# bacon205/Multimodal_eeg_fmri

Hardware: AMD Instinct MI355X
Metric: pairs_per_sec_per_node (higher is better)
Workload: dtype bf16

## Files before the change

include/mmeeg_hip.h:

```cpp
#ifndef MMEEG_HIP_H
#define MMEEG_HIP_H

#include <stdint.h>

#ifdef __cplusplus
extern "C" {
#endif

typedef struct ihipStream_t* hipStream_t;

#define MM_ABI_VERSION 5

const char* mm_last_error(void);
int mm_abi_version(void);

int mm_pack_nct_bf16(const float* x, void* y, int B, int C, int T, int Cp, hipStream_t stream);
int mm_unpack_ntc_f32(const void* g, float* dx, int B, int C, int T, int Cp, hipStream_t stream);
int mm_prep_conv_weight(const float* w, void* w_fwd, void* w_dgrad, int Cout, int Cin, int k,
                        int Cinp, int Coutp, hipStream_t stream);

int mm_conv1d_fwd(const void* x, const void* w, int B, int T, int Cin, int Cout, int taps, int pad,
                  const float* scale, const float* shift, int act, const float* residual,
                  const float* pe, int pool, float* stats, float* out_f32, void* out_bf16,
                  void* out_pre, float drop_p, uint32_t drop_seed, const uint32_t* seed_epoch,
// ... 52 lines not shown
                         int B, int D, int H, int W, float drop_p, uint32_t seed, const uint32_t* seed_epoch,
                         hipStream_t stream);
int mm_bn_act_fwd(const float* y, const float* scale, const float* shift, const float* pe,
                  void* out_bf16, float* out_f32, int R, int S, int N, int act, int pool,
                  int drop_first, float drop_p, uint32_t seed, float drop2_p, uint32_t seed2,
                  const uint32_t* seed_epoch, hipStream_t stream);
int mm_bn_act_fwd_ln(const float* y, const float* scale, const float* shift, const float* pe, float* out_f32,
                     int R, int S, int act, float drop_p, uint32_t seed, float drop2_p, uint32_t seed2,
                     const uint32_t* seed_epoch, const float* ln_gamma, const float* ln_beta, float ln_eps,
                     void* ln_out_bf16, float* ln_stat, hipStream_t stream);
int mm_bn_act_bwd_reduce(const float* y, const float* out4, const void* dout_bf16,
                         const float* dout_f32, float* sums_out, int R, int S, int N, int act,
                         int pool, int drop_first, float drop_p, uint32_t seed, float drop2_p,
                         uint32_t seed2, const uint32_t* seed_epoch, hipStream_t stream);
int mm_bn_act_bwd_apply(const float* y, const float* out4, const void* dout_bf16,
                        const float* dout_f32, const float* sums, void* dy, float* dy_f32, int R,
                        int S, int N, int act, int pool, int drop_first, float drop_p, uint32_t seed,
                        float drop2_p, uint32_t seed2, const uint32_t* seed_epoch, int train, int sums_nrep, hipStream_t stream);

int mm_layernorm_fwd(const float* x, const float* gamma, const float* beta, void* out_bf16,
                     float* out_f32, float* stat, int M, int D, float eps, hipStream_t stream);
int mm_layernorm_bwd(const void* dy_bf16, const float* dy_f32, const float* x, const float* stat,
                     const float* gamma, const float* dres, float* dx, void* dx_bf16, float* dgb_repl,
                     int M, int D, float drop_p, uint32_t seed, const uint32_t* seed_epoch,
                     hipStream_t stream);
int mm_linear_dgrad_ln_bwd(const void* dy, const void* w, int M, int K, const float* x, const float* stat,
                           const float* gamma, const float* dres, float* dx, void* dx_bf16, float* dgb_repl,
                           float drop_p, uint32_t seed, const uint32_t* seed_epoch, hipStream_t stream);

int mm_conv1d_dgrad_bn_reduce(const void* dy, const void* w_dgrad, int B, int T, int Cin, int Cout, int taps, int pad,
                              void* dx_bf16, const float* y_below, const float* out4_below, float* sums_below, int act,
                              int pool, int drop_first, float drop_p, uint32_t seed, const uint32_t* seed_epoch,
                              hipStream_t stream);

int mm_linear_fwd_ln_gemm2(const void* x, const void* w, int M, int K, const float* bias, const float* residual,
                           float* out_f32, float drop_p, uint32_t seed, const uint32_t* seed_epoch,
                           const float* ln_gamma, const float* ln_beta, float ln_eps, void* ln_out_bf16, float* ln_stat,
                           const void* w2, const float* bias2, int n2, void* out2_bf16, hipStream_t stream);
int mm_linear_fwd_ln_gemm2_act(const void* x, const void* w, int M, int K, const float* bias, const float* residual,
                               float* out_f32, float drop_p, uint32_t seed, const uint32_t* seed_epoch,
                               const float* ln_gamma, const float* ln_beta, float ln_eps, void* ln_out_bf16,
                               float* ln_stat, const void* w2, const float* bias2, int n2, void* out2_bf16,
                               void* pre2_bf16, int act2, float drop2_p, uint32_t seed2, hipStream_t stream);
int mm_linear_dgrad_ln_bwd_gemm2(const void* dy, const void* w, int M, int K, const float* x, const float* stat,
                                 const float* gamma, const float* dres, float* dx, void* dx_bf16, float* dgb_repl,
                                 float drop_p, uint32_t seed, const uint32_t* seed_epoch, const void* w2, void* do_bf16,
                                 int dres_rows_per_sample, hipStream_t stream);
int mm_linear_dgrad_ln_bwd_bn_reduce(const void* dy, const void* w, int M, int K, const float* x, const float* stat,
                                     const float* gamma, const float* dres, float* dx, float* dgb_repl,
                                     const uint32_t* seed_epoch, const float* y_below, const float* out4_below,
                                     float* sums_below, int act, float bn_drop_p, uint32_t bn_seed, float bn_drop2_p,
                                     uint32_t bn_seed2, hipStream_t stream);

int mm_bn_act_bwd_reduce_bcast(const float* y, const float* out4, const float* dout_rows, float scale, float* sums_out,
                               int R, int S, int N, int act, float drop_p, uint32_t seed, const uint32_t* seed_epoch,
                               hipStream_t stream);
int mm_bn_act_bwd_apply_bcast(const float* y, const float* out4, const float* dout_rows, float scale, const float* sums,
                              void* dy, int R, int S, int N, int act, float drop_p, uint32_t seed,
                              const uint32_t* seed_epoch, int train, int sums_nrep, hipStream_t stream);

int mm_pooled_head_bwd_rows(const float* dout, const void* z_pre_bf16, const float* W, void* dz_bf16, float* rows_out,
                            void* dx_bf16, int B, int L, int D, int N, int act, float drop_p, uint32_t seed,
                            float emit_drop_p, uint32_t emit_seed, const uint32_t* seed_epoch, hipStream_t stream);

int mm_attn_fwd(const void* qkv, void* out, float* lse, int B, int L, int H, int head_dim,
                float scale, float drop_p, uint32_t seed, const uint32_t* seed_epoch,
// ... 160 lines not shown
```

multimodal_eeg_fmri_amd/csrc/common.h:

```cpp
#pragma once
#include <hip/hip_runtime.h>
#include <stdint.h>

typedef __bf16 bf16;
typedef __attribute__((ext_vector_type(8))) __bf16 bf16x8;
typedef __attribute__((ext_vector_type(4))) __bf16 bf16x4;
typedef __attribute__((ext_vector_type(2))) __bf16 bf16x2;
typedef __attribute__((ext_vector_type(16))) float f32x16;
typedef __attribute__((ext_vector_type(4))) float f32x4;
typedef __attribute__((ext_vector_type(4))) short s16x4;

#define MM_OK 0
#define MM_ERR_ARG (-1)
#define MM_ERR_LAUNCH (-2)
#define MM_ERR_UNSUPPORTED (-3)

#define MM_ACT_NONE 0
#define MM_ACT_GELU 1
#define MM_ACT_RELU 2
#define MM_ACT_TANH 3
#define MM_ACT_SIGMOID 4

int mm_fail(int code, const char* fmt, ...);
int mm_check_launch(const char* what);
// ... 94 lines not shown
__device__ __forceinline__ uint32_t mm_eff_seed(uint32_t base, const uint32_t* epoch) {
    return epoch ? base ^ (epoch[0] * 0x85EBCA6Bu + 0xC2B2AE35u) : base;
}

template <int ACT, int POOL, class Args>
__device__ __forceinline__ void bn_dz_pair(const Args& a, float y0, float y1, float sc, float sh, float g,
                                           uint32_t i0, uint32_t i1, uint32_t io, float& dz0, float& dz1) {
    const int act = ACT >= 0 ? ACT : a.act;
    const int pool = POOL > 0 ? POOL : a.pool;
    const float z0 = y0 * sc + sh;
    if (pool == 1) {
        float m = a.thresh ? dropout_scale(a.seed, i0, a.thresh, a.inv_keep) : 1.f;
        dz0 = g * m * act_grad(z0, act);
        dz1 = 0.f;
        return;
    }
    const float z1 = y1 * sc + sh;
    float m0 = 1.f, m1 = 1.f;
    bool first;
    if (a.thresh && a.drop_first) {
        float a0 = apply_act(z0, act), a1 = apply_act(z1, act);
        m0 = dropout_scale(a.seed, i0, a.thresh, a.inv_keep);
        m1 = dropout_scale(a.seed, i1, a.thresh, a.inv_keep);
        a0 *= m0; a1 *= m1;
        first = a0 >= a1;
    } else {
        if (a.thresh) g *= dropout_scale(a.seed, io, a.thresh, a.inv_keep);
        first = z0 >= z1;
        if (act != MM_ACT_GELU || fmaxf(z0, z1) < 0.f) first = apply_act(z0, act) >= apply_act(z1, act);
    }
    const float d = g * (first ? m0 : m1) * act_grad(first ? z0 : z1, act);
    dz0 = first ? d : 0.f;
    dz1 = first ? 0.f : d;
}


#define MM_REPL 32
#define MM_ACC_REPL 16
#define MM_ACC_STAT 28
#define MM_ACC_GRAD 40
typedef long long mm_acc_t;
#define MM_ACC_POISON (1ll << 62)
#define MM_ACC_BAD ((mm_acc_t)0x8000000000000000ull)
#define MM_ACC_MAG_LIMIT ((1u << 25) - 16u)
#ifdef __HIPCC__
template <int K> __device__ __forceinline__ void acc_add(mm_acc_t* p, float v) {
    const float f = v * (float)(1ull << K);
    if (fabsf(f) < 36028797018963968.f)
        atomicAdd(reinterpret_cast<unsigned long long*>(p), (unsigned long long)__float2ll_rn(f));
    else
        atomicExch(reinterpret_cast<unsigned long long*>(p), (unsigned long long)MM_ACC_POISON);
}
template <int K> __device__ __forceinline__ mm_acc_t acc_encode(float v) {
    const float f = v * (float)(1ull << K);
    return fabsf(f) < 2305843009213693952.f ? __float2ll_rn(f) : MM_ACC_POISON;
}
__device__ __forceinline__ unsigned acc_mag(mm_acc_t v) {
    const int hi = (int)(v >> 32);
    return (unsigned)(hi < 0 ? ~hi : hi) >> 4;
}
__device__ __forceinline__ mm_acc_t acc_guard(mm_acc_t s, unsigned mag_sum) { return mag_sum >= MM_ACC_MAG_LIMIT ? MM_ACC_BAD : s; }
template <int K> __device__ __forceinline__ float acc_val(mm_acc_t s) {
    const bool bad = (unsigned long long)(s + (1ll << 61)) >= (1ull << 62);
    return bad ? __builtin_nanf("") : (float)s * (1.0f / (float)(1ull << K));
}
__device__ __forceinline__ mm_acc_t* acc_rep(float* ws, int r, size_t n) { return reinterpret_cast<mm_acc_t*>(ws) + (size_t)r * n; }
// ... 71 lines not shown
```

multimodal_eeg_fmri_amd/csrc/elementwise.hip:

```cpp
#include "common.h"

namespace {

__global__ void bn_finalize_kernel(const float* stats, const float* gamma, const float* beta,
                                   float* run_mean, float* run_var, const float* conv_bias,
                                   float* out , int N,
                                   float count, float momentum, float eps, int mode, long long* tracked) {
    const int n = blockIdx.x * blockDim.x + threadIdx.x;
    if (n >= N) return;
    if (mode == 0) {
        MmBnFin f{stats, gamma, beta, run_mean, run_var, out, tracked, count, momentum, eps, N};
        float sc, sh, mean, rstd;
        bn_fin_channel(f, n, true, sc, sh, mean, rstd);
        return;
    }
    const float mean = run_mean[n], var = run_var[n];
    const float rstd = rsqrtf(var + eps);
    const float sc = gamma[n] * rstd;
    const float cb = (mode == 1 && conv_bias) ? conv_bias[n] : 0.f;
    out[n] = sc;
    out[N + n] = beta[n] + (cb - mean) * sc;
    out[2 * N + n] = mean;
    out[3 * N + n] = rstd;
}

struct BnActArgs {
    const float* y; const float* scale; const float* shift; const float* pe;
    bf16* out_bf16; float* out_f32;
    int R, S, N, act, pool, drop_first;
    uint32_t thresh, seed; float inv_keep;
    uint32_t thresh2, seed2; float inv_keep2;
    const uint32_t* epoch;
    const float* ln_gamma = nullptr; const float* ln_beta = nullptr; float ln_eps = 0.f;
    bf16* ln_out = nullptr; float* ln_stat = nullptr;
    MmBnFin fin = {};
};

template <int ACT>
__device__ __forceinline__ float bnact_one(const BnActArgs& a, float y, float sc, float sh, uint32_t idx, bool drop_here) {
    float v = apply_act(y * sc + sh, ACT >= 0 ? ACT : a.act);
    if (drop_here && a.thresh) v *= dropout_scale(a.seed, idx, a.thresh, a.inv_keep);
    return v;
}

template <int ACT = -1, int POOL = 0, bool FIN = false>
__global__ void bn_act_fwd_kernel(BnActArgs a) {
    a.seed = mm_eff_seed(a.seed, a.epoch);
    a.seed2 = mm_eff_seed(a.seed2, a.epoch);
    if (POOL > 0) a.pool = POOL;
    __shared__ __attribute__((aligned(16))) float s_sc[FIN ? 256 : 4], s_sh[FIN ? 256 : 4];
    if (FIN) {
        for (int n = threadIdx.x; n < a.N; n += blockDim.x) {
            float sc, sh, mean, rstd;
            bn_fin_channel(a.fin, n, blockIdx.x == 0, sc, sh, mean, rstd);
            s_sc[n] = sc; s_sh[n] = sh;
        }
        __syncthreads();
    }
    const int So = a.S / a.pool;
    const unsigned nv = a.N / 4;
    const unsigned total = (unsigned)((size_t)a.R * So * nv);
    for (unsigned i = blockIdx.x * blockDim.x + threadIdx.x; i < total; i += gridDim.x * blockDim.x) {
        const unsigned rs = i / nv;
        const int n4 = (int)(i - rs * nv) * 4;
        const int so = a.pe ? (int)(rs % (unsigned)So) : 0;
        const float4 sc = FIN ? *reinterpret_cast<const float4*>(s_sc + n4) : *reinterpret_cast<const float4*>(a.scale + n4);
        const float4 sh = FIN ? *reinterpret_cast<const float4*>(s_sh + n4) : *reinterpret_cast<const float4*>(a.shift + n4);
        float o[4];
        const size_t in0 = (size_t)rs * a.pool * a.N + n4;
        const float4 y0 = *reinterpret_cast<const float4*>(a.y + in0);
        const float scs[4] = {sc.x, sc.y, sc.z, sc.w}, shs[4] = {sh.x, sh.y, sh.z, sh.w};
        const float y0s[4] = {y0.x, y0.y, y0.z, y0.w};
        const size_t oidx = (size_t)i * 4;
        if (a.pool == 2) {
            const float4 y1 = *reinterpret_cast<const float4*>(a.y + in0 + a.N);
            const float y1s[4] = {y1.x, y1.y, y1.z, y1.w};
#pragma unroll
            for (int q = 0; q < 4; ++q) {
                float m;
                const int act = ACT >= 0 ? ACT : a.act;
                const float z0 = y0s[q] * scs[q] + shs[q], z1 = y1s[q] * scs[q] + shs[q];
                if (act == MM_ACT_GELU && !(a.drop_first && a.thresh) && fmaxf(z0, z1) >= 0.f) {
                    m = gelu_erf(fmaxf(z0, z1));
                } else {
                    const float v0 = bnact_one<ACT>(a, y0s[q], scs[q], shs[q], (uint32_t)(in0 + q), a.drop_first);
                    const float v1 = bnact_one<ACT>(a, y1s[q], scs[q], shs[q], (uint32_t)(in0 + a.N + q), a.drop_first);
                    m = fmaxf(v0, v1);
                }
                if (!a.drop_first && a.thresh) m *= dropout_scale(a.seed, (uint32_t)(oidx + q), a.thresh, a.inv_keep);
                o[q] = m;
            }
        } else {
#pragma unroll
            for (int q = 0; q < 4; ++q) o[q] = bnact_one<ACT>(a, y0s[q], scs[q], shs[q], (uint32_t)(in0 + q), true);
        }
        if (a.pe) {
            const float4 p = *reinterpret_cast<const float4*>(a.pe + (size_t)so * a.N + n4);
            o[0] += p.x; o[1] += p.y; o[2] += p.z; o[3] += p.w;
        }
        if (a.thresh2)
#pragma unroll
            for (int q = 0; q < 4; ++q) o[q] *= dropout_scale(a.seed2, (uint32_t)(oidx + q), a.thresh2, a.inv_keep2);
        if (a.out_f32) *reinterpret_cast<float4*>(a.out_f32 + oidx) = make_float4(o[0], o[1], o[2], o[3]);
        if (a.out_bf16) {
            bf16x4 b = {(bf16)o[0], (bf16)o[1], (bf16)o[2], (bf16)o[3]};
            *reinterpret_cast<bf16x4*>(a.out_bf16 + oidx) = b;
        }
        if (a.ln_out) {
            const float mean = half32_sum((o[0] + o[1]) + (o[2] + o[3])) * (1.f / 128.f);
            const float d0 = o[0] - mean, d1 = o[1] - mean, d2 = o[2] - mean, d3 = o[3] - mean;
            const float rstd = rsqrtf(half32_sum((d0 * d0 + d1 * d1) + (d2 * d2 + d3 * d3)) * (1.f / 128.f) + a.ln_eps);
            const float4 g4 = *reinterpret_cast<const float4*>(a.ln_gamma + n4);
            const float4 b4 = *reinterpret_cast<const float4*>(a.ln_beta + n4);
            bf16x4 hv = {(bf16)(d0 * rstd * g4.x + b4.x), (bf16)(d1 * rstd * g4.y + b4.y),
                         (bf16)(d2 * rstd * g4.z + b4.z), (bf16)(d3 * rstd * g4.w + b4.w)};
            *reinterpret_cast<bf16x4*>(a.ln_out + oidx) = hv;
            if (a.ln_stat && n4 == 0) { a.ln_stat[2 * (size_t)rs] = mean; a.ln_stat[2 * (size_t)rs + 1] = rstd; }
        }
    }
}

struct BnBwdArgs {
    const float* y; const float* scale; const float* shift; const float* mean; const float* rstd;
    const bf16* dout_bf16; const float* dout_f32; const float* sums;
    float* sums_out; bf16* dy; float* dy_f32;
    int R, S, N, act, pool, drop_first, train;
    uint32_t thresh, seed; float inv_keep, inv_count;
// ... 623 lines not shown
```

multimodal_eeg_fmri_amd/csrc/igemm1d.hip:

```cpp
#include "common.h"

#include <cstdio>
#include <cstdlib>

namespace {


constexpr int KPAD = 8;
constexpr int A2S = 128 + KPAD;

struct BnRed {
    const float* y = nullptr;
    const float* out4 = nullptr;
    float* sums = nullptr;
    int act = 0, pool = 1, drop_first = 0;
    uint32_t thresh = 0, seed = 0;
    float inv_keep = 1.f;
    const uint32_t* epoch = nullptr;
    uint32_t thresh2 = 0, seed2 = 0;
    float inv_keep2 = 1.f;
};

struct EpiArgs {
    const float* scale;
    const float* shift;
    const float* residual;
    const float* pe;
    float* stats;
    float* out_f32;
    bf16* out_bf16;
    bf16* out_pre;
    int act;
    int pool;
    uint32_t drop_thresh;
    uint32_t drop_seed;
    float drop_inv_keep;
    const uint32_t* drop_epoch;
    const bf16* gradz;
    int gradz_act;
    const float* ln_x;
    const float* ln_stat;
    const float* ln_gamma;
    float* ln_dgb;
    float* pool_out;
    int pool_rows;
    float pool_scale;
    bf16* lnf_out;
    float* lnf_stat;
    const float* lnf_gamma;
    const float* lnf_beta;
    float lnf_eps;
    BnRed bn;
    const bf16* w2 = nullptr;
    bf16* out2 = nullptr;
    const float* bias2 = nullptr;
    int n2 = 128;
    int act2 = 0;
    uint32_t thresh2 = 0, seed2 = 0; float inv_keep2 = 1.f;
    bf16* pre2 = nullptr;
    int res_rows = 0;
};

struct ConvArgs {
    const bf16* x;
    const bf16* w;
    int B, T, Cin, Cout, taps, pad;
    EpiArgs e;
    float* partial = nullptr;
    int csplit = 0;
};

enum : unsigned { EF_RES = 1, EF_PE = 2, EF_PRE = 4, EF_GRADZ = 8, EF_STATS = 16, EF_POOLOUT = 32, EF_LNF = 64, EF_POOL2 = 128,
                  EF_DROP = 256, EF_SCALE = 512, EF_F32 = 1024, EF_BF16 = 2048, EF_SHIFT = 4096, EF_LNBWD = 8192,
                  EF_BNRED = 16384, EF_BNPOOL2 = 32768 ,
                  EF_GEMM2 = 1u << 28, EF_ANY = 0xFFFFFFFFu };
static unsigned epi_mask(const EpiArgs& e) {
    return (e.residual ? EF_RES : 0) | (e.pe ? EF_PE : 0) | (e.out_pre ? EF_PRE : 0) | (e.gradz ? EF_GRADZ : 0) | (e.stats ? EF_STATS : 0) |
           (e.pool_out ? EF_POOLOUT : 0) | (e.lnf_out ? EF_LNF : 0) | (e.pool == 2 ? EF_POOL2 : 0) | (e.drop_thresh ? EF_DROP : 0) |
           (e.scale ? EF_SCALE : 0) | (e.out_f32 ? EF_F32 : 0) | (e.out_bf16 ? EF_BF16 : 0) | (e.shift ? EF_SHIFT : 0) | (e.ln_x ? EF_LNBWD : 0) |
           ((unsigned)e.act << 16) | ((unsigned)(e.gradz ? e.gradz_act : 0) << 20) |
           (e.bn.y ? (EF_BNRED | (e.bn.pool == 2 ? EF_BNPOOL2 : 0) | ((unsigned)e.bn.act << 24)) : 0) | (e.w2 ? EF_GEMM2 : 0);
}


template <int BM, int BN, unsigned FEAT>
__device__ __forceinline__ void epilogue_rows(const float* Cs, const EpiArgs& e, int tid, int b, int t0, int T,
                                              int n0, int N, float* sstat, bf16* a2 = nullptr) {
#pragma clang fp contract(off)
    constexpr bool ANY = FEAT == EF_ANY;
#define EF_ON(bit, runtime) (ANY ? (bool)(runtime) : ((FEAT & (bit)) != 0))
    const int act = ANY ? e.act : (int)((FEAT >> 16) & 15u);
    const int gradz_act = ANY ? e.gradz_act : (int)((FEAT >> 20) & 15u);
    constexpr int LDC = BN + 4;
    constexpr int CG = BN / 4;
    constexpr int RPP = 256 / CG;
    const int cg = tid % CG, rr = tid / CG;
    const int n = n0 + cg * 4;
    const bool nok = n < N;
    float4 sc = make_float4(1.f, 1.f, 1.f, 1.f), sh = make_float4(0.f, 0.f, 0.f, 0.f);
    if (nok) {
        if (EF_ON(EF_SCALE, e.scale)) sc = *reinterpret_cast<const float4*>(e.scale + n);
        if (EF_ON(EF_SHIFT, e.shift)) sh = *reinterpret_cast<const float4*>(e.shift + n);
    }
    const float scs[4] = {sc.x, sc.y, sc.z, sc.w}, shs[4] = {sh.x, sh.y, sh.z, sh.w};
    float s1[4] = {0, 0, 0, 0}, s2[4] = {0, 0, 0, 0}, pp[4] = {0, 0, 0, 0};
    const bool drop = EF_ON(EF_DROP, e.drop_thresh);
    const uint32_t dseed = drop ? mm_eff_seed(e.drop_seed, e.drop_epoch) : 0u;
    const int step = ANY ? e.pool : ((FEAT & EF_POOL2) ? 2 : 1);
    const int To = T / step;
    for (int r0 = rr * step; r0 < BM; r0 += RPP * step) {
        float o[4] = {-INFINITY, -INFINITY, -INFINITY, -INFINITY};
        bool any = false;
        for (int q = 0; q < step; ++q) {
            const int row = r0 + q, t = t0 + row;
// ... 312 lines not shown
                const size_t idx = (row0 + row) * e.n2 + n;
                const float v = e.bias2 ? c2[r] + bias : c2[r];
                if (e.pre2) e.pre2[idx] = (bf16)v;
                float val = apply_act(v, e.act2);
                if (e.thresh2) val = __builtin_fmaf(val, dropout_scale(dseed, (uint32_t)idx, e.thresh2, e.inv_keep2), 0.f);
                orow[(size_t)row * e.n2] = (bf16)val;
            }
        }
    }
}

template <int BM, int BN, int WM, int WN, int KCT, unsigned FEAT, int TAPS>
__global__ __launch_bounds__(256, 2) void conv1d_fwd_kernel(ConvArgs a) {
    if (TAPS > 0) a.taps = TAPS;
    constexpr int TM = BM / (WM * 32);
    constexpr int TN = BN / (WN * 32);
    static_assert(WM * WN == 4, "4 waves");
    constexpr int AS = KCT + KPAD;
    constexpr int SEGS = KCT / 8;
    extern __shared__ __attribute__((aligned(16))) char smem[];

    const int tid = threadIdx.x;
    const int lane = tid & 63;
    const int wave = tid >> 6;
    const int wm = wave / WN, wn = wave % WN;
    const int tilesT = (a.T + BM - 1) / BM;
    const int b = blockIdx.x / tilesT;
    const int t0 = (blockIdx.x % tilesT) * BM;
    const int n0 = blockIdx.y * BN;
    const int arows = BM + a.taps - 1;
    bf16* As = reinterpret_cast<bf16*>(smem);
    bf16* Ws = As + arows * AS;

    f32x16 acc[TM][TN];
#pragma unroll
    for (int i = 0; i < TM; ++i)
#pragma unroll
        for (int j = 0; j < TN; ++j)
#pragma unroll
            for (int r = 0; r < 16; ++r) acc[i][j][r] = 0.f;

    const bf16* xb = a.x + (size_t)b * a.T * a.Cin;
    const int lr = lane & 31, lh = lane >> 5;
    const int wrows = BN * a.taps;
    const int wvalid = (a.Cout - n0) * a.taps;

    constexpr bool MERGE = BM == 32;
    constexpr int NA = MERGE ? 2 : 4, NB = 8;
    const bf16* wb = a.w + (size_t)n0 * a.taps * a.Cin;
    const int nA = arows * SEGS, nW = wrows * SEGS;
    auto load_a = [&](int s, int c0) {
        const int r = s / SEGS, sg = s % SEGS;
        const int t = t0 - a.pad + r;
        return (s < nA && t >= 0 && t < a.T) ? *reinterpret_cast<const uint4*>(xb + (size_t)t * a.Cin + c0 + sg * 8)
                                             : make_uint4(0, 0, 0, 0);
    };
    auto load_w = [&](int s, int c0) {
        const int r = s / SEGS, sg = s % SEGS;
        return (s < nW && r < wvalid) ? *reinterpret_cast<const uint4*>(wb + (size_t)r * a.Cin + c0 + sg * 8)
                                      : make_uint4(0, 0, 0, 0);
    };
    const int c_lo = a.partial ? (int)blockIdx.z * a.csplit : 0;
    const int c_hi = a.partial ? min(a.Cin, c_lo + a.csplit) : a.Cin;
    for (int c0 = c_lo; c0 < c_hi; c0 += KCT) {
        if (c0 != c_lo) __syncthreads();
        if constexpr (MERGE) {
            uint4 va[NA], vw[NB];
#pragma unroll
            for (int i = 0; i < NA; ++i) va[i] = load_a(i * 256 + tid, c0);
#pragma unroll
            for (int i = 0; i < NB; ++i) vw[i] = load_w(i * 256 + tid, c0);
#pragma unroll
            for (int i = 0; i < NA; ++i) {
                const int s = i * 256 + tid;
                if (s < nA) *reinterpret_cast<uint4*>(As + (s / SEGS) * AS + (s % SEGS) * 8) = va[i];
            }
#pragma unroll
            for (int i = 0; i < NB; ++i) {
                const int s = i * 256 + tid;
                if (s < nW) *reinterpret_cast<uint4*>(Ws + (s / SEGS) * AS + (s % SEGS) * 8) = vw[i];
            }
        }
        for (int base = MERGE ? NA * 256 : 0; base < nA; base += NA * 256) {
            uint4 v[NA];
#pragma unroll
            for (int i = 0; i < NA; ++i) v[i] = load_a(base + i * 256 + tid, c0);
#pragma unroll
            for (int i = 0; i < NA; ++i) {
                const int s = base + i * 256 + tid;
                if (s < nA) *reinterpret_cast<uint4*>(As + (s / SEGS) * AS + (s % SEGS) * 8) = v[i];
            }
        }
        for (int base = MERGE ? NB * 256 : 0; base < nW; base += NB * 256) {
            uint4 v[NB];
#pragma unroll
            for (int i = 0; i < NB; ++i) v[i] = load_w(base + i * 256 + tid, c0);
#pragma unroll
            for (int i = 0; i < NB; ++i) {
                const int s = base + i * 256 + tid;
                if (s < nW) *reinterpret_cast<uint4*>(Ws + (s / SEGS) * AS + (s % SEGS) * 8) = v[i];
            }
        }
        __syncthreads();
        for (int tap = 0; tap < a.taps; ++tap) {
#pragma unroll
            for (int ks = 0; ks < KCT; ks += 16) {
                bf16x8 af[TM], bfr[TN];
#pragma unroll
                for (int i = 0; i < TM; ++i) {
                    const int row = (wm * TM + i) * 32 + lr + tap;
                    af[i] = *reinterpret_cast<const bf16x8*>(As + row * AS + ks + lh * 8);
                }
#pragma unroll
                for (int j = 0; j < TN; ++j) {
                    const int nl = (wn * TN + j) * 32 + lr;
                    bfr[j] = *reinterpret_cast<const bf16x8*>(Ws + (nl * a.taps + tap) * AS + ks + lh * 8);
// ... 774 lines not shown
    a.e.pool_out = nullptr; a.e.pool_rows = 0; a.e.pool_scale = 0.f;
    a.e.lnf_out = nullptr; a.e.lnf_stat = nullptr; a.e.lnf_gamma = nullptr; a.e.lnf_beta = nullptr; a.e.lnf_eps = 0.f;
    return 0;
}

int mm_conv1d_dgrad_bn_reduce(const void* dy, const void* w_dgrad, int B, int T, int Cin, int Cout, int taps, int pad,
                              void* dx_bf16, const float* y_below, const float* out4_below, float* sums_below, int act,
                              int pool, int drop_first, float drop_p, uint32_t seed, const uint32_t* seed_epoch,
                              hipStream_t st) {
    MM_REQUIRE(dy && w_dgrad && dx_bf16 && y_below && out4_below && sums_below, "conv1d_dgrad_bn_reduce: null");
    MM_REQUIRE(B > 0 && T > 0 && Cout > 0 && taps >= 1 && taps <= 9 && pad >= 0 && pad < taps, "conv1d_dgrad_bn_reduce: bad dims");
    MM_REQUIRE(Cin > 0 && Cin % 16 == 0 && Cout % 4 == 0, "conv1d_dgrad_bn_reduce: Cin=%d (x16) Cout=%d (x4)", Cin, Cout);
    MM_REQUIRE(taps > 1 || Cout <= 64, "conv1d_dgrad_bn_reduce: the fused reduce runs on the 64 x 64 tile (taps > 1 or Cout <= 64)");
    MM_REQUIRE(pool == 1 || pool == 2, "conv1d_dgrad_bn_reduce: pool=%d", pool);
    MM_REQUIRE(drop_p >= 0.f && drop_p < 1.f, "conv1d_dgrad_bn_reduce: drop_p");
    MM_REQUIRE((size_t)B * T * pool * Cout < (1ull << 32), "conv1d_dgrad_bn_reduce: 32-bit dropout indices");
    ConvArgs a;
    a.x = (const bf16*)dy; a.w = (const bf16*)w_dgrad;
    a.B = B; a.T = T; a.Cin = Cin; a.Cout = Cout; a.taps = taps; a.pad = pad;
    a.e.scale = nullptr; a.e.shift = nullptr; a.e.residual = nullptr; a.e.pe = nullptr; a.e.stats = nullptr;
    a.e.out_f32 = nullptr; a.e.out_bf16 = (bf16*)dx_bf16; a.e.out_pre = nullptr;
    a.e.act = 0; a.e.pool = 1;
    a.e.drop_thresh = 0u; a.e.drop_seed = 0u; a.e.drop_epoch = nullptr; a.e.drop_inv_keep = 1.f;
    a.e.gradz = nullptr; a.e.gradz_act = 0;
    a.e.ln_x = nullptr; a.e.ln_stat = nullptr; a.e.ln_gamma = nullptr; a.e.ln_dgb = nullptr;
    a.e.pool_out = nullptr; a.e.pool_rows = 0; a.e.pool_scale = 0.f;
    a.e.lnf_out = nullptr; a.e.lnf_stat = nullptr; a.e.lnf_gamma = nullptr; a.e.lnf_beta = nullptr; a.e.lnf_eps = 0.f;
    a.e.bn.y = y_below; a.e.bn.out4 = out4_below; a.e.bn.sums = sums_below;
    a.e.bn.act = act; a.e.bn.pool = pool; a.e.bn.drop_first = drop_first;
    a.e.bn.thresh = drop_p > 0.f ? (uint32_t)((double)drop_p * 4294967296.0) : 0u;
    a.e.bn.seed = seed; a.e.bn.inv_keep = drop_p > 0.f ? 1.f / (1.f - drop_p) : 1.f;
    a.e.bn.epoch = seed_epoch;
    return conv1d_dispatch(a, st);
}

static int linear128_fwd(const void* x, const void* w, int M, int K, const float* bias, const float* residual,
                         float* out_f32, float drop_p, uint32_t seed, const uint32_t* seed_epoch, float* pool_out,
                         int rows_per_group, const float* ln_gamma, const float* ln_beta, float ln_eps, void* ln_out,
                         float* ln_stat, hipStream_t st, const void* w2 = nullptr, const float* bias2 = nullptr, int n2 = 0,
                         void* out2 = nullptr, int act2 = 0, float drop2_p = 0.f, uint32_t seed2 = 0, void* pre2 = nullptr) {
    MM_REQUIRE(x && w && out_f32 && M > 0 && M % 32 == 0 && K > 0 && K % 16 == 0, "linear128_fwd: M=%d (x32) K=%d (x16)", M, K);
    MM_REQUIRE(drop_p >= 0.f && drop_p < 1.f, "linear128_fwd: drop_p");
    MM_REQUIRE(!pool_out || (rows_per_group > 0 && rows_per_group % 32 == 0 && M % rows_per_group == 0),
               "linear128_fwd: rows_per_group=%d must be a multiple of 32 dividing M=%d", rows_per_group, M);
    MM_REQUIRE(!ln_out || (ln_gamma && ln_beta), "linear128_fwd: LayerNorm parameters");
    ConvArgs a;
    a.x = (const bf16*)x; a.w = (const bf16*)w;
    a.B = 1; a.T = M; a.Cin = K; a.Cout = 128; a.taps = 1; a.pad = 0;
    a.e.scale = nullptr; a.e.shift = bias; a.e.residual = residual; a.e.pe = nullptr; a.e.stats = nullptr;
    a.e.out_f32 = out_f32; a.e.out_bf16 = nullptr; a.e.out_pre = nullptr;
    a.e.act = 0; a.e.pool = 1;
    a.e.drop_thresh = drop_p > 0.f ? (uint32_t)((double)drop_p * 4294967296.0) : 0u;
    a.e.drop_seed = seed; a.e.drop_epoch = seed_epoch;
    a.e.drop_inv_keep = drop_p > 0.f ? 1.0f / (1.0f - drop_p) : 1.f;
    a.e.gradz = nullptr; a.e.gradz_act = 0;
    a.e.ln_x = nullptr; a.e.ln_stat = nullptr; a.e.ln_gamma = nullptr; a.e.ln_dgb = nullptr;
    a.e.pool_out = pool_out; a.e.pool_rows = pool_out ? rows_per_group : 0;
    a.e.pool_scale = pool_out ? 1.f / (float)rows_per_group : 0.f;
    a.e.lnf_out = (bf16*)ln_out; a.e.lnf_stat = ln_stat; a.e.lnf_gamma = ln_gamma; a.e.lnf_beta = ln_beta; a.e.lnf_eps = ln_eps;
    if (w2) {
        MM_REQUIRE(ln_out && out2 && n2 > 0 && n2 % 128 == 0, "linear128_fwd: the second GEMM needs the LayerNorm rows, an output and n2 %% 128 == 0 (n2=%d)", n2);
        MM_REQUIRE(drop2_p >= 0.f && drop2_p < 1.f && (size_t)M * n2 < (1ull << 32), "linear128_fwd: second GEMM dropout / 32-bit indices");
        a.e.w2 = (const bf16*)w2; a.e.bias2 = bias2; a.e.n2 = n2; a.e.out2 = (bf16*)out2;
        a.e.act2 = act2; a.e.pre2 = (bf16*)pre2;
        a.e.thresh2 = drop2_p > 0.f ? (uint32_t)((double)drop2_p * 4294967296.0) : 0u;
        a.e.seed2 = seed2; a.e.inv_keep2 = drop2_p > 0.f ? 1.0f / (1.0f - drop2_p) : 1.f;
// ... 338 lines not shown
```

multimodal_eeg_fmri_amd/ops.py:

```python
from __future__ import annotations

import math
import os
import weakref
from typing import Dict, List, Optional, Tuple

import torch

from . import _hip

ACT = {"none": 0, "gelu": 1, "relu": 2, "tanh": 3, "sigmoid": 4}
_BF = torch.bfloat16
_F32 = torch.float32


def _need_gpu(*tensors):
    for t in tensors:
        if t is not None and not t.is_cuda:
            raise _hip.HipLibraryError(
                "multimodal_eeg_fmri_amd runs on the MI355X HIP path only: got a CPU tensor "
                "(no CPU / eager-PyTorch fallback is provided)")
    _hip.load()


# ... 350 lines not shown


ATTN_HEAD_DIMS = tuple(range(16, 65, 8))


def attn_entry(d_model: int, nhead: int, which: str) -> str:
    dh = d_model // nhead if nhead > 0 else 0
    if nhead <= 0 or d_model % nhead or dh not in ATTN_HEAD_DIMS:
        raise ValueError(f"self-attention: (d_model, nhead) = ({d_model}, {nhead}) gives a head dim the kernels do not run; "
                         f"supported head dims: {', '.join(map(str, ATTN_HEAD_DIMS))}")
    return f"mm_attn_{which}" if dh == 32 else f"mm_attn_{which}_hd"


def attn_mask_per_head(mask, B: int, nhead: int, L: int) -> int:
    if mask is None or mask.dim() == 2:
        return 0
    if tuple(mask.shape) != (B * nhead, L, L):
        raise ValueError(f"attn_mask: the 3-D form must be (batch * heads, L, L) = ({B * nhead}, {L}, {L}), got {tuple(mask.shape)}")
    return 1


def additive_attn_mask(mask, L: int, like: torch.Tensor):
    if mask is None:
        return None
    if mask.dim() not in (2, 3) or tuple(mask.shape[-2:]) != (L, L):
        raise ValueError(f"attn_mask: expected (L, L) or (batch * heads, L, L) with L = {L}, got {tuple(mask.shape)}")
    if mask.dtype == torch.bool:
        m = torch.zeros(tuple(mask.shape), dtype=_F32, device=like.device)
        m.masked_fill_(mask.to(like.device), float("-inf"))
        return m
    return mask.to(device=like.device, dtype=_F32).contiguous()


def conv_bn_act(xb: torch.Tensor, conv, bn, *, act="gelu", pool=1, training=False, drop_p=0.0,
                drop_first=True, pe=None, pe_drop_p=0.0, want_f32=False, want_bf16=True, need_dgrad=False,
                save=None, next_norm=None):
    save = training if save is None else save
    k = conv.kernel_size[0]
    pad = conv.padding[0]
    cout = conv.out_channels
    wf, _, cinp, _ = weights.get(conv.weight, need_dgrad)
    assert xb.shape[2] == cinp, (xb.shape, cinp)
    B, T, _ = xb.shape
    if not save:
        out4 = bn_fold_eval(bn, conv.bias)
        r = igemm(xb, wf, k, pad, cout, scale=out4[0], shift=out4[1], act=act, pe=pe, pool=pool,
                  out_f32=want_f32, out_bf16=want_bf16)
        return r, None
    stats = _zeros((REPL, 2, cout), xb) if training else None
    y = igemm(xb, wf, k, pad, cout, shift=conv.bias, stats=stats, out_f32=True, out_bf16=False)["f32"]
    fold = training and act == "gelu" and cout <= 256 and isinstance(bn.running_mean, torch.Tensor)
    fin = None
    if fold:
        fin, out4 = bn_fin_desc(bn, stats, B * T)
    else:
        out4 = bn_finalize_train(bn, stats, B * T) if training else bn_fold_eval(bn, None)
    if not training:
        drop_p = pe_drop_p = 0.0
    seed = _next_seed() if drop_p > 0 else 0
    seed2 = _next_seed() if pe_drop_p > 0 else 0
    of = _empty((B, T // pool, cout), _F32, xb) if want_f32 else None
    ob = _empty((B, T // pool, cout), _BF, xb) if want_bf16 else None
    prenorm = None
    if next_norm is not None and cout == 128 and pool == 1 and want_f32 and not want_bf16 and drop_first \
            and tuple(next_norm.normalized_shape) == (128,):
        hn = _empty((B * T, cout), _BF, xb)
        stn = _empty((B * T, 2), _F32, xb)
        if fold:
            import ctypes
            _hip.call("mm_bn_act_fwd_ln_fin", y, ctypes.addressof(fin), pe, of, B, T, ACT[act], float(drop_p), seed,
                      float(pe_drop_p), seed2, EP(), next_norm.weight, next_norm.bias, float(next_norm.eps), hn, stn)
        else:
            _hip.call("mm_bn_act_fwd_ln", y, out4[0], out4[1], pe, of, B, T, ACT[act], float(drop_p), seed,
                      float(pe_drop_p), seed2, EP(), next_norm.weight, next_norm.bias, float(next_norm.eps), hn, stn)
        prenorm = (hn, stn)
    elif fold:
        import ctypes
        _hip.call("mm_bn_act_fwd_fin", y, ctypes.addressof(fin), pe, ob, of, B, T, cout, ACT[act], pool,
                  1 if drop_first else 0, float(drop_p), seed, float(pe_drop_p), seed2, EP())
    else:
        _hip.call("mm_bn_act_fwd", y, out4[0], out4[1], pe, ob, of, B, T, cout, ACT[act], pool,
                  1 if drop_first else 0, float(drop_p), seed, float(pe_drop_p), seed2, EP())
    saved = dict(xb=xb, y=y, out4=out4, act=act, pool=pool, drop_p=drop_p, seed=seed,
                 drop2=(float(pe_drop_p), seed2), drop_first=drop_first, conv=conv, bn=bn, train=training)
    return {"f32": of, "bf16": ob, "pre": None, "prenorm": prenorm}, saved


def transformer_block_fwd(x: torch.Tensor, blk, training: bool, need_dgrad: bool = False,
                          save: Optional[bool] = None, pool_out: Optional[torch.Tensor] = None,
                          prenorm=None, next_norm=None, mask=None, next_blk=None):
    B, L, D = x.shape
    M = B * L
    save = training if save is None else save
    p = blk.dropout.p if training else 0.0
    x2 = x.view(M, D)
    fuse_ln = D == 128 and M % 32 == 0
    h1, st1 = prenorm[:2] if prenorm is not None else layernorm(x2, blk.norm1, save)
    if prenorm is not None and len(prenorm) > 2:
        qkv = prenorm[2]
    else:
        qkv = linear_rows(h1, blk.self_attn.in_proj_weight, blk.self_attn.in_proj_bias,
                          need_dgrad=need_dgrad)["bf16"]
    pa = float(blk.self_attn.dropout) if training else 0.0
    sa = _next_seed() if pa > 0 else 0
    o, lse = attention(qkv.view(B, L, 3 * D), blk.nhead, save, pa, sa, mask)
    s1 = _next_seed() if p > 0 else 0
    f1 = None
    s2 = None
    if fuse_ln:
        wf, _, cinp, _ = weights.get(blk.self_attn.out_proj.weight, need_dgrad)
        x1 = _empty((M, D), _F32, x)
        h2 = _empty((M, D), _BF, x)
        st2 = _empty((M, 2), _F32, x) if save else None
        w1, _, c1, _ = weights.get(blk.linear1.weight, need_dgrad)
        n1 = blk.linear1.weight.shape[0]
        if c1 == 128 and n1 % 128 == 0 and M * n1 < (1 << 32) and not _NO_FFN1_FUSE:
            s2 = _next_seed() if p > 0 else 0
            g1 = _empty((M, n1), _BF, x)
# ... 88 lines not shown
    if L > pe.shape[0]:
        raise ValueError(f"sequence length {L} exceeds PositionalEncoding max_len {pe.shape[0]}")
    return pe[:L, 0, :].contiguous()


def _encoder_tail_impl(m, h, training: bool, need_dgrad: bool, save: bool, prenorm=None, stages=None):
    blocks = []
    B, L, D = h.shape
    nblk = len(m.transformer_layers)
    pooled = _zeros((B, 2 * D), h) if nblk and L % 32 == 0 and D == 128 else None
    layers = list(m.transformer_layers)
    for i, blk in enumerate(layers):
        if i < nblk - 1:
            h, s, prenorm = transformer_block_fwd(h, blk, training, need_dgrad, save=save, prenorm=prenorm,
                                                  next_norm=layers[i + 1].norm1, next_blk=layers[i + 1])
        else:
            h, s = transformer_block_fwd(h, blk, training, need_dgrad, save=save, pool_out=pooled, prenorm=prenorm)
        blocks.append(s)
        if stages is not None:
            stages[f"block{i}"] = h.clone()
    out, s = pooled_head_fwd(h, m.output_proj[2], training=training, drop_p=m.drop_p, need_dgrad=need_dgrad,
                             save=save, pooled_f32=pooled)
    return out, blocks, s, h


def _erp_forward_impl(m, x: torch.Tensor, training: bool, need_dgrad: bool, save=None, xb=None, stages=None):
    cl = m.conv_layers
    save = training if save is None else save
    p = m.drop_p if training else 0.0
    if xb is None:
        xb = pack_nct(x)
    saved = []
    saved_in = []
    r, s = conv_bn_act(xb, cl[0], cl[1], training=training, drop_p=p, need_dgrad=need_dgrad, save=save)
    saved.append(s)
    saved_in.append(r["bf16"])
    r, s = conv_bn_act(r["bf16"], cl[4], cl[5], pool=2, training=training, drop_p=p,
                       drop_first=False, need_dgrad=need_dgrad, save=save)
    saved.append(s)
    saved_in.append(r["bf16"])
    L = r["bf16"].shape[1]
    r, s = conv_bn_act(r["bf16"], cl[9], cl[10], training=training, drop_p=p,
                       pe=pe_table(m.pos_encoder, L), pe_drop_p=(m.pos_encoder.dropout.p if training else 0.0),
                       want_f32=True, want_bf16=False, need_dgrad=need_dgrad, save=save,
                       next_norm=m.transformer_layers[0].norm1 if len(m.transformer_layers) else None)
    saved.append(s)
    if stages is not None:
        stages["conv1"], stages["conv2"] = saved_in[0].clone(), saved_in[1].clone()
        stages["pos"] = r["f32"].clone()
        if not save:
            wf3 = weights.get(cl[9].weight, need_dgrad)[0]
            o4 = bn_fold_eval(cl[10], cl[9].bias)
            stages["conv3"] = igemm(saved_in[1], wf3, cl[9].kernel_size[0], cl[9].padding[0], cl[9].out_channels,
                                    scale=o4[0], shift=o4[1], act="gelu", out_f32=True, out_bf16=False)["f32"]
    out, blocks, s, h = _encoder_tail_impl(m, r["f32"], training, need_dgrad, save, prenorm=r.get("prenorm"), stages=stages)
    return out, dict(convs=saved, blocks=blocks, head=s, x_shape=tuple(x.shape), tokens=h)


def erp_encoder_forward(m, x: torch.Tensor) -> torch.Tensor:
    _need_gpu(x)
    if m.training or _wants_grad(m, x):
        from .autograd import ErpEncoderFn
        return ErpEncoderFn.run(m, x)
    with torch.no_grad():
        return _erp_forward_impl(m, x.float(), False, False)[0]


def _wants_grad(m, x) -> bool:
    return torch.is_grad_enabled() and (x.requires_grad or any(p.requires_grad for p in m.parameters()))


def add_positional(x, pe, drop_p, training):
    _need_gpu(x)
    if x.dim() != 3:
        raise ValueError("PositionalEncoding: expected a 3-D input (batch, seq, d_model) or (seq, 1, d_model)")
    L = x.size(1) if x.size(1) != 1 else x.size(0)
    if L > pe.shape[0]:
        raise ValueError(f"sequence length {L} exceeds PositionalEncoding max_len {pe.shape[0]}")
    from .autograd import AddPositionalFn
# ... 738 lines not shown
```

Baseline: 41800.

## Fuse BatchNorm apply, GELU, pool and dropout into next conv's input staging

In training, the BN-apply/activation/pool/dropout pass of the first two conv blocks is deferred. The next implicit-GEMM conv then reads the raw fp32 pre-BN output and applies BN finalize, GELU, optional max-pool and dropout while staging its A tile into shared memory. It also writes the bf16 activation once, from blockIdx.y==0 tiles, for the backward pass. This removes a separate elementwise kernel launch and its bf16 round trip per block. In exchange, the conv reads fp32 data (twice as much when pooled) and recomputes the activation for every output-channel tile, and the new path is restricted to 64-row tiles.

```diff
diff --git a/include/mmeeg_hip.h b/include/mmeeg_hip.h
--- a/include/mmeeg_hip.h
+++ b/include/mmeeg_hip.h
@@ -108,6 +108,9 @@
                               void* dx_bf16, const float* y_below, const float* out4_below, float* sums_below, int act,
                               int pool, int drop_first, float drop_p, uint32_t seed, const uint32_t* seed_epoch,
                               hipStream_t stream);
+int mm_conv1d_fwd_bn_in(const float* y_below, const void* bn_fin_host, int pool, int drop_first, float drop_p,
+                        uint32_t seed, void* act_bf16, const void* w, int B, int T, int Cin, int Cout, int taps, int pad,
+                        const float* shift, float* stats, float* out_f32, const uint32_t* seed_epoch, hipStream_t stream);
 
 int mm_linear_fwd_ln_gemm2(const void* x, const void* w, int M, int K, const float* bias, const float* residual,
                            float* out_f32, float drop_p, uint32_t seed, const uint32_t* seed_epoch,
diff --git a/multimodal_eeg_fmri_amd/csrc/common.h b/multimodal_eeg_fmri_amd/csrc/common.h
--- a/multimodal_eeg_fmri_amd/csrc/common.h
+++ b/multimodal_eeg_fmri_amd/csrc/common.h
@@ -150,6 +150,33 @@
     const float d = g * (first ? m0 : m1) * act_grad(first ? z0 : z1, act);
     dz0 = first ? d : 0.f;
     dz1 = first ? 0.f : d;
+}
+
+template <int ACT, int POOL, class Args>
+__device__ __forceinline__ float bn_act_fwd_one(const Args& a, float y0, float y1, float sc, float sh,
+                                                uint32_t i0, uint32_t i1, uint32_t io) {
+    const int act = ACT >= 0 ? ACT : a.act;
+    const int pool = POOL > 0 ? POOL : a.pool;
+    const float z0 = y0 * sc + sh;
+    if (pool == 1) {
+        float v = apply_act(z0, act);
+        if (a.thresh) v *= dropout_scale(a.seed, i0, a.thresh, a.inv_keep);
+        return v;
+    }
+    const float z1 = y1 * sc + sh;
+    float m;
+    if (act == MM_ACT_GELU && !(a.drop_first && a.thresh) && fmaxf(z0, z1) >= 0.f) {
+        m = gelu_erf(fmaxf(z0, z1));
+    } else {
+        float v0 = apply_act(z0, act), v1 = apply_act(z1, act);
+        if (a.drop_first && a.thresh) {
+            v0 *= dropout_scale(a.seed, i0, a.thresh, a.inv_keep);
+            v1 *= dropout_scale(a.seed, i1, a.thresh, a.inv_keep);
+        }
+        m = fmaxf(v0, v1);
+    }
+    if (!a.drop_first && a.thresh) m *= dropout_scale(a.seed, io, a.thresh, a.inv_keep);
+    return m;
 }
 
 
diff --git a/multimodal_eeg_fmri_amd/csrc/elementwise.hip b/multimodal_eeg_fmri_amd/csrc/elementwise.hip
--- a/multimodal_eeg_fmri_amd/csrc/elementwise.hip
+++ b/multimodal_eeg_fmri_amd/csrc/elementwise.hip
@@ -35,13 +35,6 @@
     bf16* ln_out = nullptr; float* ln_stat = nullptr;
     MmBnFin fin = {};
 };
-
-template <int ACT>
-__device__ __forceinline__ float bnact_one(const BnActArgs& a, float y, float sc, float sh, uint32_t idx, bool drop_here) {
-    float v = apply_act(y * sc + sh, ACT >= 0 ? ACT : a.act);
-    if (drop_here && a.thresh) v *= dropout_scale(a.seed, idx, a.thresh, a.inv_keep);
-    return v;
-}
 
 template <int ACT = -1, int POOL = 0, bool FIN = false>
 __global__ void bn_act_fwd_kernel(BnActArgs a) {
@@ -76,23 +69,12 @@
             const float4 y1 = *reinterpret_cast<const float4*>(a.y + in0 + a.N);
             const float y1s[4] = {y1.x, y1.y, y1.z, y1.w};
 #pragma unroll
-            for (int q = 0; q < 4; ++q) {
-                float m;
-                const int act = ACT >= 0 ? ACT : a.act;
-                const float z0 = y0s[q] * scs[q] + shs[q], z1 = y1s[q] * scs[q] + shs[q];
-                if (act == MM_ACT_GELU && !(a.drop_first && a.thresh) && fmaxf(z0, z1) >= 0.f) {
-                    m = gelu_erf(fmaxf(z0, z1));
-                } else {
-                    const float v0 = bnact_one<ACT>(a, y0s[q], scs[q], shs[q], (uint32_t)(in0 + q), a.drop_first);
-                    const float v1 = bnact_one<ACT>(a, y1s[q], scs[q], shs[q], (uint32_t)(in0 + a.N + q), a.drop_first);
-                    m = fmaxf(v0, v1);
-                }
-                if (!a.drop_first && a.thresh) m *= dropout_scale(a.seed, (uint32_t)(oidx + q), a.thresh, a.inv_keep);
-                o[q] = m;
-            }
+            for (int q = 0; q < 4; ++q)
+                o[q] = bn_act_fwd_one<ACT, 2>(a, y0s[q], y1s[q], scs[q], shs[q], (uint32_t)(in0 + q), (uint32_t)(in0 + a.N + q),
+                                              (uint32_t)(oidx + q));
         } else {
 #pragma unroll
-            for (int q = 0; q < 4; ++q) o[q] = bnact_one<ACT>(a, y0s[q], scs[q], shs[q], (uint32_t)(in0 + q), true);
+            for (int q = 0; q < 4; ++q) o[q] = bn_act_fwd_one<ACT, 1>(a, y0s[q], y0s[q], scs[q], shs[q], (uint32_t)(in0 + q), 0u, 0u);
         }
         if (a.pe) {
             const float4 p = *reinterpret_cast<const float4*>(a.pe + (size_t)so * a.N + n4);
diff --git a/multimodal_eeg_fmri_amd/csrc/igemm1d.hip b/multimodal_eeg_fmri_amd/csrc/igemm1d.hip
--- a/multimodal_eeg_fmri_amd/csrc/igemm1d.hip
+++ b/multimodal_eeg_fmri_amd/csrc/igemm1d.hip
@@ -19,6 +19,16 @@
     const uint32_t* epoch = nullptr;
     uint32_t thresh2 = 0, seed2 = 0;
     float inv_keep2 = 1.f;
+};
+
+struct BnIn {
+    const float* y = nullptr;
+    MmBnFin fin = {};
+    bf16* act_out = nullptr;
+    int act = MM_ACT_GELU, pool = 1, drop_first = 1;
+    uint32_t thresh = 0, seed = 0;
+    float inv_keep = 1.f;
+    const uint32_t* epoch = nullptr;
 };
 
 struct EpiArgs {
@@ -59,6 +69,7 @@
     uint32_t thresh2 = 0, seed2 = 0; float inv_keep2 = 1.f;
     bf16* pre2 = nullptr;
     int res_rows = 0;
+    BnIn bnin;
 };
 
 struct ConvArgs {
@@ -73,13 +84,14 @@
 enum : unsigned { EF_RES = 1, EF_PE = 2, EF_PRE = 4, EF_GRADZ = 8, EF_STATS = 16, EF_POOLOUT = 32, EF_LNF = 64, EF_POOL2 = 128,
                   EF_DROP = 256, EF_SCALE = 512, EF_F32 = 1024, EF_BF16 = 2048, EF_SHIFT = 4096, EF_LNBWD = 8192,
                   EF_BNRED = 16384, EF_BNPOOL2 = 32768 ,
-                  EF_GEMM2 = 1u << 28, EF_ANY = 0xFFFFFFFFu };
+                  EF_GEMM2 = 1u << 28, EF_BNIN = 1u << 29, EF_BNIN_POOL2 = 1u << 30, EF_ANY = 0xFFFFFFFFu };
 static unsigned epi_mask(const EpiArgs& e) {
     return (e.residual ? EF_RES : 0) | (e.pe ? EF_PE : 0) | (e.out_pre ? EF_PRE : 0) | (e.gradz ? EF_GRADZ : 0) | (e.stats ? EF_STATS : 0) |
            (e.pool_out ? EF_POOLOUT : 0) | (e.lnf_out ? EF_LNF : 0) | (e.pool == 2 ? EF_POOL2 : 0) | (e.drop_thresh ? EF_DROP : 0) |
            (e.scale ? EF_SCALE : 0) | (e.out_f32 ? EF_F32 : 0) | (e.out_bf16 ? EF_BF16 : 0) | (e.shift ? EF_SHIFT : 0) | (e.ln_x ? EF_LNBWD : 0) |
            ((unsigned)e.act << 16) | ((unsigned)(e.gradz ? e.gradz_act : 0) << 20) |
-           (e.bn.y ? (EF_BNRED | (e.bn.pool == 2 ? EF_BNPOOL2 : 0) | ((unsigned)e.bn.act << 24)) : 0) | (e.w2 ? EF_GEMM2 : 0);
+           (e.bn.y ? (EF_BNRED | (e.bn.pool == 2 ? EF_BNPOOL2 : 0) | ((unsigned)e.bn.act << 24)) : 0) | (e.w2 ? EF_GEMM2 : 0) |
+           (e.bnin.y ? (EF_BNIN | (e.bnin.pool == 2 ? EF_BNIN_POOL2 : 0)) : 0);
 }
 
 
@@ -458,6 +470,19 @@
     bf16* As = reinterpret_cast<bf16*>(smem);
     bf16* Ws = As + arows * AS;
 
+    constexpr bool BNIN = FEAT != EF_ANY && (FEAT & EF_BNIN) != 0;
+    constexpr int BPOOL = (FEAT & EF_BNIN_POOL2) && BNIN ? 2 : 1;
+    __shared__ __attribute__((aligned(16))) float s_bn[BNIN ? 512 : 1];
+    if constexpr (BNIN) {
+        a.e.bnin.seed = mm_eff_seed(a.e.bnin.seed, a.e.bnin.epoch);
+        for (int n = tid; n < a.Cin; n += 256) {
+            float sc, sh, mean, rstd;
+            bn_fin_channel(a.e.bnin.fin, n, blockIdx.x == 0 && blockIdx.y == 0, sc, sh, mean, rstd);
+            s_bn[n] = sc; s_bn[256 + n] = sh;
+        }
+        __syncthreads();
+    }
+
     f32x16 acc[TM][TN];
 #pragma unroll
     for (int i = 0; i < TM; ++i)
@@ -472,6 +497,7 @@
     const int wvalid = (a.Cout - n0) * a.taps;
 
     constexpr bool MERGE = BM == 32;
+    static_assert(!(MERGE && BNIN), "the BatchNorm-applying staging runs on the 64-row tiles");
     constexpr int NA = MERGE ? 2 : 4, NB = 8;
     const bf16* wb = a.w + (size_t)n0 * a.taps * a.Cin;
     const int nA = arows * SEGS, nW = wrows * SEGS;
@@ -486,6 +512,50 @@
         return (s < nW && r < wvalid) ? *reinterpret_cast<const uint4*>(wb + (size_t)r * a.Cin + c0 + sg * 8)
                                       : make_uint4(0, 0, 0, 0);
     };
+    auto stage_bn = [&](int base, int c0) __attribute__((always_inline)) {
+        constexpr int NY = 2 * BPOOL;
+        const int Tin = a.T * BPOOL;
+        const float* yb = a.e.bnin.y + (size_t)b * Tin * a.Cin;
+        float4 v[NA][NY];
+#pragma unroll
+        for (int i = 0; i < NA; ++i) {
+            const int s = base + i * 256 + tid;
+            const int r = s / SEGS, sg = s % SEGS;
+            const int t = t0 - a.pad + r;
+            const bool ok = s < nA && t >= 0 && t < a.T;
+            const float* p = yb + (ok ? (size_t)t * BPOOL * a.Cin + c0 + sg * 8 : 0);
+#pragma unroll
+            for (int j = 0; j < BPOOL; ++j) {
+                v[i][2 * j] = *reinterpret_cast<const float4*>(p + j * a.Cin);
+                v[i][2 * j + 1] = *reinterpret_cast<const float4*>(p + j * a.Cin + 4);
+            }
+        }
+#pragma unroll
+        for (int i = 0; i < NA; ++i) {
+            const int s = base + i * 256 + tid;
+            if (s >= nA) continue;
+            const int r = s / SEGS, sg = s % SEGS;
+            const int t = t0 - a.pad + r;
+            const int c = c0 + sg * 8;
+            bf16x8 h;
+#pragma unroll
+            for (int q = 0; q < 8; ++q) h[q] = (bf16)0.f;
+            if (t >= 0 && t < a.T) {
+                const float y0s[8] = {v[i][0].x, v[i][0].y, v[i][0].z, v[i][0].w, v[i][1].x, v[i][1].y, v[i][1].z, v[i][1].w};
+                const float4 u0 = v[i][NY - 2], u1 = v[i][NY - 1];
+                const float y1s[8] = {u0.x, u0.y, u0.z, u0.w, u1.x, u1.y, u1.z, u1.w};
+                const uint32_t i0 = (uint32_t)(((size_t)b * Tin + (size_t)t * BPOOL) * a.Cin + c);
+                const uint32_t io = (uint32_t)(((size_t)b * a.T + t) * a.Cin + c);
+#pragma unroll
+                for (int q = 0; q < 8; ++q)
+                    h[q] = (bf16)bn_act_fwd_one<MM_ACT_GELU, BPOOL>(a.e.bnin, y0s[q], y1s[q], s_bn[c + q], s_bn[256 + c + q],
+                                                                    i0 + q, i0 + a.Cin + q, io + q);
+                if (blockIdx.y == 0 && r >= a.pad && r < a.pad + BM)
+                    *reinterpret_cast<bf16x8*>(a.e.bnin.act_out + ((size_t)b * a.T + t) * a.Cin + c) = h;
+            }
+            *reinterpret_cast<bf16x8*>(As + r * AS + sg * 8) = h;
+        }
+    };
     const int c_lo = a.partial ? (int)blockIdx.z * a.csplit : 0;
     const int c_hi = a.partial ? min(a.Cin, c_lo + a.csplit) : a.Cin;
     for (int c0 = c_lo; c0 < c_hi; c0 += KCT) {
@@ -508,6 +578,10 @@
             }
         }
         for (int base = MERGE ? NA * 256 : 0; base < nA; base += NA * 256) {
+            if constexpr (BNIN) {
+                stage_bn(base, c0);
+                continue;
+            }
             uint4 v[NA];
 #pragma unroll
             for (int i = 0; i < NA; ++i) v[i] = load_a(base + i * 256 + tid, c0);
@@ -1348,6 +1422,29 @@
     a.e.bn.seed = seed; a.e.bn.inv_keep = drop_p > 0.f ? 1.f / (1.f - drop_p) : 1.f;
     a.e.bn.epoch = seed_epoch;
     return conv1d_dispatch(a, st);
+}
+
+int mm_conv1d_fwd_bn_in(const float* y_below, const void* bn_fin_host, int pool, int drop_first, float drop_p, uint32_t seed,
+                        void* act_bf16, const void* w, int B, int T, int Cin, int Cout, int taps, int pad, const float* shift,
+                        float* stats, float* out_f32, const uint32_t* seed_epoch, hipStream_t st) {
+    MM_REQUIRE(y_below && act_bf16 && shift && stats && out_f32, "conv1d_fwd_bn_in: null");
+    ConvArgs a;
+    int rc = conv1d_fwd_args(a, act_bf16, w, B, T, Cin, Cout, taps, pad, nullptr, shift, 0, nullptr, nullptr, 1, stats, out_f32,
+                             nullptr, nullptr, 0.f, 0u, seed_epoch, nullptr, 0);
+    if (rc) return rc;
+    MM_REQUIRE(bn_fin_from_host(a.e.bnin.fin, bn_fin_host, Cin), "conv1d_fwd_bn_in: incomplete mm_bn_fin_t (null pointer or count < 1)");
+    MM_REQUIRE(taps > 1 && Cin % 64 == 0 && Cin <= 256, "conv1d_fwd_bn_in: taps=%d (> 1), Cin=%d (a multiple of 64, <= 256)", taps, Cin);
+    MM_REQUIRE(conv1d_splitk_slices(B, T, Cin, Cout, taps) == 1, "conv1d_fwd_bn_in: a split-K shape");
+    MM_REQUIRE(pool == 1 || pool == 2, "conv1d_fwd_bn_in: pool=%d", pool);
+    MM_REQUIRE(drop_p >= 0.f && drop_p < 1.f, "conv1d_fwd_bn_in: drop_p");
+    MM_REQUIRE((size_t)B * T * pool * Cin < (1ull << 32), "conv1d_fwd_bn_in: 32-bit dropout indices");
+    a.e.bnin.y = y_below; a.e.bnin.act_out = (bf16*)act_bf16;
+    a.e.bnin.act = MM_ACT_GELU; a.e.bnin.pool = pool; a.e.bnin.drop_first = drop_first ? 1 : 0;
+    a.e.bnin.thresh = drop_p > 0.f ? (uint32_t)((double)drop_p * 4294967296.0) : 0u;
+    a.e.bnin.seed = seed; a.e.bnin.inv_keep = drop_p > 0.f ? 1.f / (1.f - drop_p) : 1.f;
+    a.e.bnin.epoch = seed_epoch;
+    if (pool == 2) return launch_fwd_feat<64, 64, 2, 2, 64, 0x001410u | EF_BNIN | EF_BNIN_POOL2, 0>(a, st);
+    return launch_fwd_feat<64, 64, 2, 2, 64, 0x001410u | EF_BNIN, 0>(a, st);
 }
 
 static int linear128_fwd(const void* x, const void* w, int M, int K, const float* bias, const float* residual,
diff --git a/multimodal_eeg_fmri_amd/ops.py b/multimodal_eeg_fmri_amd/ops.py
--- a/multimodal_eeg_fmri_amd/ops.py
+++ b/multimodal_eeg_fmri_amd/ops.py
@@ -406,23 +406,36 @@
     return mask.to(device=like.device, dtype=_F32).contiguous()
 
 
-def conv_bn_act(xb: torch.Tensor, conv, bn, *, act="gelu", pool=1, training=False, drop_p=0.0,
+def conv_bn_act(xb: Optional[torch.Tensor], conv, bn, *, act="gelu", pool=1, training=False, drop_p=0.0,
                 drop_first=True, pe=None, pe_drop_p=0.0, want_f32=False, want_bf16=True, need_dgrad=False,
-                save=None, next_norm=None):
+                save=None, next_norm=None, defer_apply=False, below=None):
     save = training if save is None else save
     k = conv.kernel_size[0]
     pad = conv.padding[0]
     cout = conv.out_channels
     wf, _, cinp, _ = weights.get(conv.weight, need_dgrad)
-    assert xb.shape[2] == cinp, (xb.shape, cinp)
-    B, T, _ = xb.shape
+    below_bf16 = None
+    if below is not None:
+        import ctypes
+        yb = below["y"]
+        B, T = yb.shape[0], yb.shape[1] // below["pool"]
+        assert save and training and yb.shape[2] == cinp, (yb.shape, cinp)
+        xb = below_bf16 = _empty((B, T, cinp), _BF, yb)
+        stats = _zeros((REPL, 2, cout), yb)
+        y = _empty((B, T, cout), _F32, yb)
+        _hip.call("mm_conv1d_fwd_bn_in", yb, ctypes.addressof(below["fin"]), below["pool"], 1 if below["drop_first"] else 0,
+                  float(below["drop_p"]), below["seed"], xb, wf, B, T, cinp, cout, k, pad, conv.bias, stats, y, EP())
+    else:
+        assert xb.shape[2] == cinp, (xb.shape, cinp)
+        B, T, _ = xb.shape
     if not save:
         out4 = bn_fold_eval(bn, conv.bias)
         r = igemm(xb, wf, k, pad, cout, scale=out4[0], shift=out4[1], act=act, pe=pe, pool=pool,
                   out_f32=want_f32, out_bf16=want_bf16)
         return r, None
-    stats = _zeros((REPL, 2, cout), xb) if training else None
-    y = igemm(xb, wf, k, pad, cout, shift=conv.bias, stats=stats, out_f32=True, out_bf16=False)["f32"]
+    if below is None:
+        stats = _zeros((REPL, 2, cout), xb) if training else None
+        y = igemm(xb, wf, k, pad, cout, shift=conv.bias, stats=stats, out_f32=True, out_bf16=False)["f32"]
     fold = training and act == "gelu" and cout <= 256 and isinstance(bn.running_mean, torch.Tensor)
     fin = None
     if fold:
@@ -433,6 +446,12 @@
         drop_p = pe_drop_p = 0.0
     seed = _next_seed() if drop_p > 0 else 0
     seed2 = _next_seed() if pe_drop_p > 0 else 0
+    if defer_apply:
+        assert fold and pe is None and pe_drop_p == 0.0, "defer_apply: train-mode GELU block without a positional table"
+        deferred = dict(y=y, fin=fin, pool=pool, drop_first=drop_first, drop_p=drop_p, seed=seed)
+        saved = dict(xb=xb, y=y, out4=out4, act=act, pool=pool, drop_p=drop_p, seed=seed,
+                     drop2=(0.0, 0), drop_first=drop_first, conv=conv, bn=bn, train=training)
+        return {"f32": None, "bf16": None, "pre": None, "prenorm": None, "deferred": deferred, "below_bf16": below_bf16}, saved
     of = _empty((B, T // pool, cout), _F32, xb) if want_f32 else None
     ob = _empty((B, T // pool, cout), _BF, xb) if want_bf16 else None
     prenorm = None
@@ -457,7 +476,14 @@
                   1 if drop_first else 0, float(drop_p), seed, float(pe_drop_p), seed2, EP())
     saved = dict(xb=xb, y=y, out4=out4, act=act, pool=pool, drop_p=drop_p, seed=seed,
                  drop2=(float(pe_drop_p), seed2), drop_first=drop_first, conv=conv, bn=bn, train=training)
-    return {"f32": of, "bf16": ob, "pre": None, "prenorm": prenorm}, saved
+    return {"f32": of, "bf16": ob, "pre": None, "prenorm": prenorm, "below_bf16": below_bf16}, saved
+
+
+def bn_in_fusable(bn, cout: int, conv_next, B: int, T_next: int) -> bool:
+    k = conv_next.kernel_size[0]
+    return (k > 1 and conv_next.in_channels == cout and cpad(cout) == cout and cout % 64 == 0 and cout <= 256
+            and isinstance(bn.running_mean, torch.Tensor)
+            and _splitk_plan(B, T_next, cout, conv_next.out_channels, k)[0] == 1)
 
 
 def transformer_block_fwd(x: torch.Tensor, blk, training: bool, need_dgrad: bool = False,
@@ -612,19 +638,22 @@
         xb = pack_nct(x)
     saved = []
     saved_in = []
-    r, s = conv_bn_act(xb, cl[0], cl[1], training=training, drop_p=p, need_dgrad=need_dgrad, save=save)
+    B, _, T = x.shape
+    f1 = save and training and bn_in_fusable(cl[1], cl[0].out_channels, cl[4], B, T)
+    f2 = f1 and bn_in_fusable(cl[5], cl[4].out_channels, cl[9], B, T // 2)
+    r1, s = conv_bn_act(xb, cl[0], cl[1], training=training, drop_p=p, need_dgrad=need_dgrad, save=save, defer_apply=f1)
     saved.append(s)
-    saved_in.append(r["bf16"])
-    r, s = conv_bn_act(r["bf16"], cl[4], cl[5], pool=2, training=training, drop_p=p,
-                       drop_first=False, need_dgrad=need_dgrad, save=save)
+    r2, s = conv_bn_act(r1["bf16"], cl[4], cl[5], pool=2, training=training, drop_p=p,
+                        drop_first=False, need_dgrad=need_dgrad, save=save, below=r1.get("deferred"), defer_apply=f2)
     saved.append(s)
-    saved_in.append(r["bf16"])
-    L = r["bf16"].shape[1]
+    saved_in.append(r2["below_bf16"] if f1 else r1["bf16"])
+    r = r2
     r, s = conv_bn_act(r["bf16"], cl[9], cl[10], training=training, drop_p=p,
-                       pe=pe_table(m.pos_encoder, L), pe_drop_p=(m.pos_encoder.dropout.p if training else 0.0),
+                       pe=pe_table(m.pos_encoder, T // 2), pe_drop_p=(m.pos_encoder.dropout.p if training else 0.0),
                        want_f32=True, want_bf16=False, need_dgrad=need_dgrad, save=save,
-                       next_norm=m.transformer_layers[0].norm1 if len(m.transformer_layers) else None)
+                       next_norm=m.transformer_layers[0].norm1 if len(m.transformer_layers) else None, below=r.get("deferred"))
     saved.append(s)
+    saved_in.append(r["below_bf16"] if f2 else r2["bf16"])
     if stages is not None:
         stages["conv1"], stages["conv2"] = saved_in[0].clone(), saved_in[1].clone()
         stages["pos"] = r["f32"].clone()
```

Measured after the change: 40720, median of 2. 2.6% lower.
